# chalharu/rust-compression

Hardware: AMD Instinct MI355X
Metric: BZip2 level-9 encode MB/s (input bytes, HBM-resident in and out: the kernels' rate; value_end_to_end is host buffer to host buffer at the C ABI) (higher is better)
Workload: dtype u8/u32

## Files before the change

rust-compression_amd/csrc/k_bwt.hip:

```cpp
#include "bzgpu.h"
#include <algorithm>
#include <atomic>
#include <cstdio>
#include <cstdlib>
#include <vector>

namespace bzgpu {
constexpr u32 kGhSpan = 8;
constexpr u32 kSymSpan = 8;

enum { SRC_TEXT = 0, SRC_PAIRS = 1, SRC_MM = 2, SRC_WALK = 3, SRC_SURV = 4, SRC_LISTG = 5,
       SRC_TEXTK = 6, SRC_WALKK = 7, SRC_MMK = 8,
       SRC_MMC = 9,
       SRC_PERJ = 10,
       SRC_PACKED = 11,
       SRC_PERJK = 12,
       SRC_WALKA = 13 };
template <int SRC> struct src_is_list {
    static constexpr bool value = (SRC == SRC_PAIRS || SRC == SRC_SURV || SRC == SRC_LISTG || SRC == SRC_PERJ || SRC == SRC_PERJK || SRC == SRC_PACKED);
};

struct KeyInfo {
    u8 bits;
    u8 chars;
// ... 2547 lines not shown
__global__ __launch_bounds__(kSortThreads) void k_link_compact(BwtArgs a, const u32 *__restrict__ VS, u32 *__restrict__ Kout, u32 *__restrict__ Vout)
{
    constexpr u32 NW = kSortThreads / 64;
    __shared__ u32 s_off, s_wsum[NW];
    u32 tile, lb;
    xcd_remap(gridDim.x, a.nb, tile, lb);
    if (lb == 0xFFFFFFFFu) return;
    const u32 cnt = a.count2[lb];
    const u32 start = tile * kSortTile;
    const u32 ntiles = (cnt + kSortTile - 1) / kSortTile;
    if (tile == 0 && threadIdx.x == 0) {
        u32 tot = 0;
        for (u32 t = 0; t < ntiles; ++t) tot += a.tile_nf[lb * kTilesPerBlock + t];
        a.count[lb] = tot;
    }
    if (start >= cnt) return;
    const size_t base = (size_t)lb * kSlot;
    if (threadIdx.x == 0) {
        u32 off = 0;
        for (u32 t = 0; t < tile; ++t) off += a.tile_nf[lb * kTilesPerBlock + t];
        s_off = off;
    }
    const u8 *gb8 = group_bytes(a, lb);
    const u32 w = threadIdx.x >> 6, l = threadIdx.x & 63u;
    const u32 wbase = start + w * 1024u;
    u64 keep[16];
    u32 xv[16];
    u32 wcount = 0;
#pragma unroll
    for (u32 r = 0; r < 16; ++r) {
        const u32 idx = wbase + r * 64u + l;
        const u32 c = idx < cnt ? idx : cnt - 1u;
        xv[r] = ld_stream(VS + base + c);
        keep[r] = __ballot(idx < cnt && gb8[c] != 1u);
        wcount += (u32)__popcll(keep[r]);
    }
    if (l == 0) s_wsum[w] = wcount;
    __syncthreads();
    u32 off = s_off;
    for (u32 k = 0; k < w; ++k) off += s_wsum[k];
    const u64 lt_mask = (l == 0) ? 0ull : (~0ull >> (64 - l));
#pragma unroll
    for (u32 r = 0; r < 16; ++r) {
        if ((keep[r] >> l) & 1ull) {
            const u32 at = off + (u32)__popcll(keep[r] & lt_mask);
            Kout[base + at] = a.R[base + xv[r]] & ~kFinalBit;
            Vout[base + at] = xv[r];
        }
        off += (u32)__popcll(keep[r]);
    }
}

__global__ __launch_bounds__(kSortThreads) void k_period_mark(BwtArgs a, u32 step, const u32 *__restrict__ K,
                                                               const u32 *__restrict__ V, u8 *__restrict__ impure)
{
    u32 tile, lb;
    xcd_remap(gridDim.x, a.nb, tile, lb);
    if (lb == 0xFFFFFFFFu) return;
    const u32 cnt = a.count[lb];
    const u32 start = tile * kSortTile;
    if (start >= cnt || a.lin_p[(size_t)lb * kPerK] == 0u) return;
    const u32 n = a.blocks[lb].n;
    const u32 kmax = per_kmax(a);
    (void)step;
    const size_t base = (size_t)lb * kSlot;
    u32 lp[kPerK];
#pragma unroll
    for (u32 i = 0; i < kPerK; ++i) lp[i] = i < kmax ? a.lin_p[(size_t)lb * kPerK + i] : 0u;
    const u32 w = threadIdx.x >> 6, l = threadIdx.x & 63u;
    const u32 first = start + w * 1024u + l;
    u32 g[16], v[16];
#pragma unroll
    for (u32 r = 0; r < 16; ++r) {
        const u32 idx = first + r * 64u;
        const u32 c = idx < cnt ? idx : cnt - 1u;
        g[r] = ld_stream(K + base + c);
        v[r] = ld_stream(V + base + c);
    }
    u32 pg0 = 0, pv0 = 0;
    if (l == 0 && first > 0 && first < cnt) {
        pg0 = K[base + first - 1];
        pv0 = V[base + first - 1];
    }
    u32 lo[16], wh[16];
    u32 act = 0, vp_lo = 0;
#pragma unroll
    for (u32 r = 0; r < 16; ++r) {
        const u32 idx = first + r * 64u;
        u32 pg = wave_shr1(g[r]), pv = wave_shr1(v[r]);
        const u32 qg = (r == 0) ? pg0 : wave_lane(g[(r + 15) & 15], 63);
        const u32 qv = (r == 0) ? pv0 : wave_lane(v[(r + 15) & 15], 63);
        if (l == 0) {
            pg = qg;
            pv = qv;
        }
        lo[r] = v[r] < pv ? v[r] : pv;
        wh[r] = kPerK;
        if (idx < cnt && idx > 0 && g[r] == pg) {
            const u32 dist = v[r] < pv ? pv - v[r] : v[r] - pv;
#pragma unroll
            for (u32 i = 0; i < kPerK; ++i)
                if (lp[i] != 0u && lp[i] == dist) wh[r] = i;
            if (wh[r] == kPerK) impure[base + g[r]] = 1;
            else {
                act |= 1u << r;
                vp_lo |= (pv == lo[r] ? 1u : 0u) << r;
            }
        }
    }
    u64 here[16];
#pragma unroll
    for (u32 r = 0; r < 16; ++r) here[r] = ((act >> r) & 1u) ? (per_mis(a, lb, wh[r])[lo[r] >> 6] & (~0ull << (lo[r] & 63u))) : 1ull;
    u32 m[16];
#pragma unroll
    for (u32 r = 0; r < 16; ++r)
        m[r] = here[r] ? ((lo[r] >> 6) << 6) + (u32)__builtin_ctzll(here[r]) : per_nxt(a, lb, wh[r])[(lo[r] >> 6) + 1u];
    u64 ltw[16];
#pragma unroll
    for (u32 r = 0; r < 16; ++r) {
        if (m[r] >= n) m[r] -= n;
        ltw[r] = ((act >> r) & 1u) ? per_lt(a, lb, wh[r])[m[r] >> 6] : 0ull;
    }
#pragma unroll
    for (u32 r = 0; r < 16; ++r) {
        if (!((act >> r) & 1u)) continue;
        const bool lo_first = (ltw[r] >> (m[r] & 63u)) & 1ull;
        if (lo_first != (((vp_lo >> r) & 1u) != 0u)) impure[base + g[r]] = 1;
    }
}

__global__ __launch_bounds__(kSortThreads) void k_block_symbols(BwtArgs a, u32 *__restrict__ inuse_bits ,
                                                                u32 *__restrict__ pair_bits )
{
    __shared__ u32 s_bits[8];
    __shared__ u32 s_pair[kPairWords];
    u32 tile, lb;
    xcd_remap(gridDim.x, a.nb, tile, lb);
    if (lb == 0xFFFFFFFFu) return;
    const BlockDesc d = a.blocks[lb];
    const u32 n = d.n;
    constexpr u32 kSpan = kSymSpan * kSortTile;
    const u32 start = tile * kSpan;
    if (start >= n) return;
    const u8 *text = a.rle + d.rle_off;
    if (threadIdx.x < 8) s_bits[threadIdx.x] = 0;
    if (pair_bits)
        for (u32 i = threadIdx.x; i < kPairWords; i += kSortThreads) s_pair[i] = 0;
    __syncthreads();
    const u32 cnt = (n - start) < kSpan ? (n - start) : kSpan;
    const uintptr_t p0 = reinterpret_cast<uintptr_t>(text + start);
    const u32 lead = (u32)(p0 & 15u);
    const uint4 *src = reinterpret_cast<const uint4 *>(p0 - lead);
    const u32 t0 = text[0];
    u64 set[4] = {0, 0, 0, 0};
    for (u32 c = threadIdx.x; c * 16u < lead + cnt; c += kSortThreads) {
        const uint4 v = src[c];
        const u32 w[4] = {v.x, v.y, v.z, v.w};
        const u32 behind = start + c * 16u + 16u - lead;
        const u32 nxt = (pair_bits && behind < n) ? (u32)text[behind] : t0;
#pragma unroll
        for (u32 k = 0; k < 16; ++k) {
            const u32 pos = c * 16u + k;
            const u32 b = (w[k >> 2] >> ((k & 3u) * 8u)) & 0xFFu;
            const bool in = pos >= lead && pos < lead + cnt;
            const u64 bit = in ? (1ull << (b & 63u)) : 0ull;
            const u32 hi = b >> 6;
#pragma unroll
            for (u32 q = 0; q < 4; ++q) set[q] |= (hi == q) ? bit : 0ull;
            if (pair_bits && in) {
                u32 b2 = (k < 15u) ? ((w[(k + 1u) >> 2] >> (((k + 1u) & 3u) * 8u)) & 0xFFu) : nxt;
                if (start + (pos - lead) + 1u == n) b2 = t0;
                const u32 pr = (b << 8) | b2;
                if (!((s_pair[pr >> 5] >> (pr & 31u)) & 1u)) atomicOr(&s_pair[pr >> 5], 1u << (pr & 31u));
            }
        }
    }
    u32 seen[8];
#pragma unroll
    for (u32 q = 0; q < 4; ++q) {
        seen[2 * q] = (u32)set[q];
        seen[2 * q + 1] = (u32)(set[q] >> 32);
    }
#pragma unroll
    for (u32 q = 0; q < 8; ++q) {
        u32 v = seen[q];
#pragma unroll
        for (u32 dd = 32; dd >= 1; dd >>= 1) v |= __shfl_xor(v, dd, 64);
        if ((threadIdx.x & 63u) == 0 && v) atomicOr(&s_bits[q], v);
    }
    __syncthreads();
    if (threadIdx.x < 8 && s_bits[threadIdx.x]) atomicOr(&inuse_bits[lb * 8 + threadIdx.x], s_bits[threadIdx.x]);
    if (pair_bits)
        for (u32 i = threadIdx.x; i < kPairWords; i += kSortThreads)
            if (s_pair[i]) atomicOr(&pair_bits[(size_t)lb * kPairWords + i], s_pair[i]);
}

__global__ __launch_bounds__(256) void k_key_params(const u32 *__restrict__ inuse_bits, const u32 *__restrict__ pair_bits,
                                                     u8 *__restrict__ sym_code, u8 *__restrict__ keyinfo)
{
    __shared__ u32 s_pairs[4];
    const u32 lb = blockIdx.x;
    const u32 *bits = inuse_bits + lb * 8;
    const u32 v = threadIdx.x;
    u32 before = 0;
    for (u32 q = 0; q < (v >> 5); ++q) before += __popc(bits[q]);
    before += __popc(bits[v >> 5] & ((1u << (v & 31u)) - 1u));
    sym_code[(size_t)lb * 256 + v] = (u8)before;
    if (pair_bits) {
        u32 mine = 0;
        for (u32 i = v; i < kPairWords; i += 256u) mine += __popc(pair_bits[(size_t)lb * kPairWords + i]);
        mine = wave_incl_sum(mine);
        if ((v & 63u) == 63u) s_pairs[v >> 6] = mine;
    }
    __syncthreads();
    if (v == 0) {
        u32 alpha = 0;
        for (u32 q = 0; q < 8; ++q) alpha += __popc(bits[q]);
        u32 nbits = 1;
        while ((1u << nbits) < alpha) ++nbits;
        u32 chars = (nbits >= 8) ? 4u : 30u / nbits;
        if (chars > 8u) chars = 8u;
        KeyInfo ki;
        ki.bits = (u8)nbits;
        ki.chars = (u8)chars;
        ki.form = 0;
        ki.pad = 0;
        if (pair_bits) {
            const u32 npairs = s_pairs[0] + s_pairs[1] + s_pairs[2] + s_pairs[3];
            u32 pbits = 1;
            while (pbits < 11u && (1u << pbits) < npairs) ++pbits;
            const u32 cpair = 2u * (30u / pbits) < 8u ? 2u * (30u / pbits) : 8u;
            if (pbits <= 10u && cpair > chars) {
                ki.bits = (u8)pbits;
                ki.chars = (u8)cpair;
                ki.form = 1;
            }
        }
        reinterpret_cast<KeyInfo *>(keyinfo)[lb] = ki;
    }
}

__global__ __launch_bounds__(kSortThreads) void k_pack_text(BwtArgs a, u8 *__restrict__ ptext)
{
    __shared__ u8 s_code[256];
    __shared__ u32 s_out[kSortTile / 32 * 10];
    __shared__ u32 s_pair[kPairWords];
    __shared__ u16 s_before[kPairWords];
    __shared__ u32 s_wsum[kSortThreads / 64];
    __shared__ u32 s_hist[2][1024];
    u32 span, lb;
    xcd_remap(gridDim.x, a.nb, span, lb);
    if (lb == 0xFFFFFFFFu) return;
    const BlockDesc d = a.blocks[lb];
    const u32 n = d.n;
    const u32 start0 = span * kGhSpan * kSortTile;
    if (n == 0 || start0 >= n + 16u) return;
    const u8 *text = a.rle + d.rle_off;
    const KeyInfo ki = reinterpret_cast<const KeyInfo *>(a.keyinfo)[lb];
    const u32 bits = ki.bits;
    const bool pairs = ki.form != 0;
    const bool count = a.gh_tiles != nullptr && counts_from_pack(ki);
    if (count)
        for (u32 i = threadIdx.x; i < 2u * 1024u; i += kSortThreads) (&s_hist[0][0])[i] = 0;
    if (pairs) {
        static_assert(kPairWords == 4 * kSortThreads, "four words of the pair map per thread");
        const uint4 w4 = reinterpret_cast<const uint4 *>(a.pair_bits + (size_t)lb * kPairWords)[threadIdx.x];
        const u32 w[4] = {w4.x, w4.y, w4.z, w4.w};
        const u32 mine = __popc(w[0]) + __popc(w[1]) + __popc(w[2]) + __popc(w[3]);
        const u32 inc = wave_incl_sum(mine);
        if ((threadIdx.x & 63u) == 63u) s_wsum[threadIdx.x >> 6] = inc;
        __syncthreads();
        u32 run = inc - mine;
        for (u32 k = 0; k < (threadIdx.x >> 6); ++k) run += s_wsum[k];
#pragma unroll
        for (u32 q = 0; q < 4; ++q) {
            s_pair[threadIdx.x * 4u + q] = w[q];
            s_before[threadIdx.x * 4u + q] = (u16)run;
            run += __popc(w[q]);
        }
    } else {
        for (u32 i = threadIdx.x; i < 256; i += kSortThreads) s_code[i] = a.sym_code[(size_t)lb * 256 + i];
    }
    __syncthreads();
    u8 *s_bytes = reinterpret_cast<u8 *>(s_out);
    u32 *const hist = s_hist[threadIdx.x & 1u];
#pragma unroll 1
    for (u32 sp = 0; sp < kGhSpan; ++sp) {
        const u32 tile = span * kGhSpan + sp, start = tile * kSortTile;
        if (start >= n + 16u) break;
#pragma unroll
        for (u32 h = 0; h < 2; ++h) {
            const u32 g = h * kSortThreads + threadIdx.x;
            const u32 i0 = start + g * 8u;
            u32 lo = 0, hi = 0, ninth = 0;
            if (i0 + 9u <= n) {
                const uintptr_t p = reinterpret_cast<uintptr_t>(text + i0);
                const u32 *ap = reinterpret_cast<const u32 *>(p & ~(uintptr_t)3);
                const u32 w0 = ap[0], w1 = ap[1], w2 = ap[2];
                lo = __builtin_amdgcn_alignbyte(w1, w0, (u32)(p & 3u));
                hi = __builtin_amdgcn_alignbyte(w2, w1, (u32)(p & 3u));
                ninth = (w2 >> (8u * (u32)(p & 3u))) & 0xFFu;
            } else if (i0 < n + 16u) {
                for (u32 q = 0; q < 9; ++q) {
                    const u32 i = i0 + q;
                    const u32 c = (i < n + 16u + (q >> 3)) ? (u32)text[i < n ? i : (i - n) % n] : 0u;
                    if (q < 4) lo |= c << (8u * q);
                    else if (q < 8) hi |= c << (8u * (q - 4u));
                    else ninth = c;
                }
            }
            u64 va = 0, vb = 0;
#pragma unroll
            for (u32 q = 0; q < 8; ++q) {
                const u32 byte = ((q < 4 ? lo >> (8u * q) : hi >> (8u * (q - 4u)))) & 0xFFu;
                u32 code;
                if (pairs) {
                    const u32 b2 = q == 7 ? ninth : (((q + 1 < 4 ? lo >> (8u * (q + 1)) : hi >> (8u * (q + 1 - 4u)))) & 0xFFu);
                    const u32 pr = (byte << 8) | b2;
                    code = (u32)s_before[pr >> 5] + __popc(s_pair[pr >> 5] & ((1u << (pr & 31u)) - 1u));
                    if (i0 + q >= n + 16u) code = 0;
                    if (count && i0 + q < n) atomicAdd(&hist[code], 1u);
                } else {
                    code = s_code[byte];
                }
                if (q < 4) va = (va << bits) | (u64)code;
                else vb = (vb << bits) | (u64)code;
            }
            for (u32 k = 0; k < bits; ++k) {
                const u32 sh = 8u * (bits - 1u - k), half = 4u * bits;
                u32 o = sh >= half ? (u32)(va >> (sh - half)) : ((u32)(vb >> sh) | (u32)(va << (half - sh)));
                s_bytes[g * bits + k] = (u8)o;
            }
        }
        __syncthreads();
        u32 *dst = reinterpret_cast<u32 *>(ptext + (size_t)lb * kPtSlot + (size_t)tile * 1024u * bits);
        for (u32 i = threadIdx.x; i < 256u * bits; i += kSortThreads) dst[i] = s_out[i];
        __syncthreads();
    }
    if (count) {
        u32 *out = a.gh_tiles + ((size_t)lb * kTilesPerBlock + span) * 3 * kMaxBins;
        for (u32 i = threadIdx.x; i < 1024u; i += kSortThreads) out[i] = s_hist[0][i] + s_hist[1][i];
    }
}

int KernelProf::begin(hipStream_t st, int id, u64 nbytes)
{
    if (!on) return -1;
// ... 519 lines not shown
```

rust-compression_amd/csrc/k_huff.hip:

```cpp
#include "bzgpu.h"
#include <cstdlib>

namespace bzgpu {

constexpr u32 kHuffThreads = 512;

__device__ __forceinline__ u32 weight_add(u32 x, u32 y)
{
    const u32 dx = x & 0xFFu, dy = y & 0xFFu;
    return ((x & 0xFFFFFF00u) + (y & 0xFFFFFF00u)) | (1u + (dx > dy ? dx : dy));
}

__device__ void down_heap(u32 *buf, u32 nn, u32 len)
{
    const u32 tmp = buf[nn];
    u32 leaf = (nn << 1) + 1;
    while (leaf < len) {
        if (leaf + 1 < len && buf[buf[leaf]] > buf[buf[leaf + 1]]) leaf += 1;
        if (buf[tmp] < buf[buf[leaf]]) break;
        buf[nn] = buf[leaf];
        nn = leaf;
        leaf = (nn << 1) + 1;
    }
    buf[nn] = tmp;
// ... 737 lines not shown
#pragma unroll
    for (int t = 0; t < 6; ++t) last[t] = -1000000;
    for (u32 g = g_lo; g < g_hi; ++g) {
        const u32 v = selector[g];
#pragma unroll
        for (int t = 0; t < 6; ++t)
            if ((u32)t == v) last[t] = (int)g;
    }
    int start_last[6];
#pragma unroll
    for (int t = 0; t < 6; ++t) {
        const int inc = wave_incl_max32(last[t]);
        if (lane == 63) s_scan[wave] = (u32)inc;
        __syncthreads();
        int carry = -1000000;
        for (u32 k = 0; k < wave; ++k) carry = (int)s_scan[k] > carry ? (int)s_scan[k] : carry;
        const int prev = __shfl_up(inc, 1, 64);
        int ex = (lane == 0) ? -1000000 : prev;
        ex = ex > carry ? ex : carry;
        start_last[t] = (ex < 0) ? -(t + 1) : ex;
        __syncthreads();
    }
    u32 my_bits = 0;
    {
        int cur[6];
#pragma unroll
        for (int t = 0; t < 6; ++t) cur[t] = start_last[t];
        for (u32 g = g_lo; g < g_hi; ++g) {
            const u32 v = selector[g];
            int lv = 0;
#pragma unroll
            for (int t = 0; t < 6; ++t)
                if ((u32)t == v) lv = cur[t];
            u32 pos = 0;
#pragma unroll
            for (int t = 0; t < 6; ++t) pos += (cur[t] > lv) ? 1u : 0u;
#pragma unroll
            for (int t = 0; t < 6; ++t)
                if ((u32)t == v) cur[t] = (int)g;
            my_bits += pos + 1u;
        }
    }
    u32 sel_off, sel_total;
    {
        const u32 inc = wave_incl_sum(my_bits);
        if (lane == 63) s_scan[wave] = inc;
        __syncthreads();
        u32 carry = 0, tot = 0;
        for (u32 k = 0; k < kHuffThreads / 64; ++k) {
            if (k < wave) carry += s_scan[k];
            tot += s_scan[k];
        }
        sel_off = carry + inc - my_bits;
        sel_total = tot;
        __syncthreads();
    }
    const u32 tab_bit0 = sel_bit0 + sel_total;
    if (tab_lane) {
        const u8 *l = s_len[tb];
        u32 nb = 5, curr = l[0];
        for (u32 i = 0; i < alpha; ++i) {
            const u32 li = l[i];
            nb += 2u * (li > curr ? li - curr : curr - li) + 1u;
            curr = li;
        }
        s_first[tb][0] = nb;
    }
    __syncthreads();
    u32 tab_off[7];
    tab_off[0] = tab_bit0;
    for (u32 t = 0; t < 6; ++t) tab_off[t + 1] = tab_off[t] + (t < group_num ? s_first[t][0] : 0u);
    const u32 hb = tab_off[group_num];
    for (u32 w = tid; w <= (hb >> 5); w += kHuffThreads) stream[w] = 0;
    __syncthreads();
    auto put = [&](u32 bitpos, u32 v, u32 nbits) {
        const u32 w = bitpos >> 5, o = bitpos & 31u;
        const unsigned long long x = (unsigned long long)v << (64u - o - nbits);
        atomicOr(&stream[w], (u32)(x >> 32));
        if ((u32)x) atomicOr(&stream[w + 1], (u32)x);
    };
    if (tid == 0) {
        put(0, 0x314159u, 24);
        put(24, 0x265359u, 24);
        put(48, a.crc[lb], 32);
        put(81, a.orig_ptr[lb], 24);
        put(105, in_use16, 16);
        u32 bp = 121;
        for (u32 i = 0; i < 16; ++i) {
            const u32 half = (ubits[i >> 1] >> ((i & 1u) * 16u)) & 0xFFFFu;
            if (half) {
                put(bp, __brev(half) >> 16, 16);
                bp += 16;
            }
        }
        put(bp, group_num, 3);
        put(bp + 3, n_selectors, 15);
    }
    {
        int cur[6];
#pragma unroll
        for (int t = 0; t < 6; ++t) cur[t] = start_last[t];
        u32 bp = sel_bit0 + sel_off;
        for (u32 g = g_lo; g < g_hi; ++g) {
            const u32 v = selector[g];
            int lv = 0;
#pragma unroll
            for (int t = 0; t < 6; ++t)
                if ((u32)t == v) lv = cur[t];
            u32 pos = 0;
#pragma unroll
            for (int t = 0; t < 6; ++t) pos += (cur[t] > lv) ? 1u : 0u;
#pragma unroll
            for (int t = 0; t < 6; ++t)
                if ((u32)t == v) cur[t] = (int)g;
            put(bp, (1u << (pos + 1u)) - 2u, pos + 1u);
            bp += pos + 1u;
        }
    }
    if (tab_lane) {
        const u8 *l = s_len[tb];
        u32 bp = tab_off[tb];
        u32 curr = l[0];
        put(bp, curr, 5);
        bp += 5;
        for (u32 i = 0; i < alpha; ++i) {
            const u32 li = l[i];
            while (curr < li) { put(bp, 2, 2); bp += 2; curr += 1; }
            while (curr > li) { put(bp, 3, 2); bp += 2; curr -= 1; }
            bp += 1;
        }
    }
    if (tid == 0) {
        bo.header_bits = hb;
        bo.pad = used_ranges | (sel_total << 5);
        bo.total_bits = (u64)hb + payload_bits;
        bo.group_num = group_num;
        bo.n_selectors = n_selectors;
        bo.max_len = max_len;
        bo.lm_tables = s_lm[0] + s_lm[1] + s_lm[2] + s_lm[3] + s_lm[4] + s_lm[5];
        bo.crc = a.crc[lb];
        bo.orig_ptr = a.orig_ptr[lb];
        if ((u64)hb + payload_bits + 96u > (u64)kStreamWords * 32u) atomicExch(a.error_flag, 1u);
    }
    {
        const u64 tb = (u64)hb + payload_bits;
        u32 w0 = (hb >> 5) + 1u;
        u32 w1 = (u32)(tb >> 5) + 2u;
        if (w1 > kStreamWords) w1 = kStreamWords;
        for (u32 w = w0 + tid; w < w1; w += kHuffThreads) stream[w] = 0;
    }
    BZ_HT(3)
}

__global__ __launch_bounds__(256) void k_emit_payload(HuffArgs a)
{
    __shared__ u32 s_code[6 * kMaxAlpha];
    __shared__ u32 s_sym[256 * kGSize / 2];
    const u32 lb = blockIdx.y;
    const BlockOut &bo = a.out[lb];
    const u32 mtf_count = bo.mtf_count;
    const u32 n_selectors = bo.n_selectors;
    const u32 g0 = blockIdx.x * 256u;
    if (g0 >= n_selectors) return;
    const u32 *code_len = a.code_len + (size_t)lb * 6 * kMaxAlpha;
    for (u32 i = threadIdx.x; i < 6 * kMaxAlpha; i += 256u) s_code[i] = code_len[i];
    const u16 *mtf = a.mtf + (size_t)lb * a.mtf_stride;
    stage_symbols(s_sym, mtf, g0, mtf_count);
    __syncthreads();
    const u32 g = g0 + threadIdx.x;
    if (g >= n_selectors) return;
    const u32 gs = g * kGSize;
    const u32 cnt = (gs + kGSize < mtf_count) ? kGSize : mtf_count - gs;
    const u32 *my = s_sym + threadIdx.x * (kGSize / 2);
    const u32 *tab = s_code + (u32)a.selector[(size_t)lb * kSelStride + g] * kMaxAlpha;
    const u32 bitpos = bo.header_bits + a.group_bitoff[(size_t)lb * kGboStride + g];
    u32 *stream = a.stream + (size_t)lb * kStreamWords;
    u32 widx = bitpos >> 5;
    u32 nacc = bitpos & 31u;
    u64 acc = 0;
    bool first = true;
    for (u32 i = 0; i < cnt; ++i) {
        const u32 cl = tab[(my[i >> 1] >> ((i & 1u) * 16u)) & 0xFFFFu];
        const u32 len = cl >> 24, code = cl & 0xFFFFFFu;
        acc |= (u64)code << (64u - nacc - len);
        nacc += len;
        if (nacc >= 32u) {
            const u32 word = (u32)(acc >> 32);
            if (first) {
                atomicOr(&stream[widx], word);
                first = false;
            } else {
                stream[widx] = word;
            }
            ++widx;
            acc <<= 32;
            nacc -= 32u;
        }
    }
    if (nacc) atomicOr(&stream[widx], (u32)(acc >> 32));
}

constexpr u32 kSweepThreads = 256;
constexpr u32 kSweepTilesX = 11;
constexpr u32 kTabArena = 6 * (3 * kMaxAlpha + 4);

__device__ __forceinline__ u32 huff_group_num(u32 mtf_count)
{
    if (mtf_count < 200) return 2;
    if (mtf_count < 600) return 3;
    if (mtf_count < 1200) return 4;
    if (mtf_count < 2400) return 5;
    return 6;
}

__device__ __forceinline__ void lm_wave_sync()
{
    __builtin_amdgcn_fence(__ATOMIC_ACQ_REL, "workgroup");
    __builtin_amdgcn_wave_barrier();
}
__device__ void lm_code_lengths_wave(const u32 *rfreq, u32 n, u32 *scr, u32 scr_words, u32 row, u8 *out, u32 lane)
{
    const u32 lim = kLim;
    u32 *map = scr;
    u32 *sfreq = map + kMaxAlpha;
    u32 *c = sfreq + kMaxAlpha;
    u32 *misc = c + kMaxAlpha;
    u32 *max_elem = misc, *b = misc + 20, *cur = misc + 40;
    u32 *val = misc + 64 + kMaxAlpha;
    u32 *ty = val + lim * row;
    u32 *w = scr + scr_words - kMaxAlpha;
    for (u32 i = lane; i < n; i += 64u) {
        const u32 f = rfreq[i];
        w[i] = (f > 1u ? f : 1u) << 8;
    }
    lm_wave_sync();
    for (u32 i = lane; i < n; i += 64u) {
        const u32 f = w[i];
        u32 r = 0;
        for (u32 q = 0; q < n; ++q) {
            const u32 x = w[q];
            r += (x > f || (x == f && q < i)) ? 1u : 0u;
        }
        sfreq[r] = f;
        map[r] = i;
    }
    if (lane == 0) {
        for (u32 j = 0; j < lim; ++j) { max_elem[j] = 0; b[j] = 0; cur[j] = 0; }
        u32 excess = (1u << lim) - n;
        const u32 half = 1u << (lim - 1);
        max_elem[lim - 1] = n;
        for (u32 j = 0; j < lim; ++j) {
            if (excess >= half) {
                b[j] = 1;
                excess -= half;
            }
            excess <<= 1;
            if (lim >= 2 + j) max_elem[lim - 2 - j] = max_elem[lim - 1 - j] / 2 + n;
        }
        max_elem[0] = b[0];
        for (u32 j = 1; j < lim; ++j)
            if (max_elem[j] > 2 * max_elem[j - 1] + b[j]) max_elem[j] = 2 * max_elem[j - 1] + b[j];
    }
    lm_wave_sync();
    for (u32 j = 0; j < lim; ++j)
        for (u32 t = lane; t < max_elem[j]; t += 64u) { val[j * row + t] = 0; ty[j * row + t] = 0; }
    for (u32 i = lane; i < n; i += 64u) c[i] = lim;
    lm_wave_sync();
    for (u32 t = lane; t < n && t < max_elem[lim - 1]; t += 64u) {
        val[(lim - 1) * row + t] = sfreq[t];
        ty[(lim - 1) * row + t] = t;
    }
    if (lane == 0 && b[lim - 1] == 1) {
        c[0] -= 1;
        cur[lim - 1] += 1;
    }
    lm_wave_sync();
    const u32 last_leaf = sfreq[n - 1];
    for (u32 j = lim - 1; j > 0;) {
        const u32 next0 = cur[j], me = max_elem[j], cap = max_elem[j - 1];
        const u32 K = (me > next0 + 1u) ? (me - next0) / 2u : 0u;
        u32 *vj = val + j * row, *dv = val + (j - 1) * row, *dt = ty + (j - 1) * row;
        for (u32 k0 = 0; k0 < K; k0 += 64u) {
            const u32 k = k0 + lane;
            u32 pk = 0;
            if (k < K) pk = weight_add(vj[next0 + 2u * k], vj[next0 + 2u * k + 1u]);
            lm_wave_sync();
            if (k < K) vj[k] = pk;
        }
        lm_wave_sync();
        for (u32 k = lane; k < K; k += 64u) {
            const u32 pk = vj[k];
            if (pk > last_leaf) {
                u32 lo = 0, hi = n;
                while (lo < hi) {
                    const u32 mid = (lo + hi) >> 1;
                    if (sfreq[mid] >= pk) lo = mid + 1u;
                    else hi = mid;
                }
                const u32 pos = k + lo;
                if (pos < cap) {
                    dv[pos] = pk;
                    dt[pos] = n;
                }
            }
        }
        for (u32 i = lane; i < n; i += 64u) {
            const u32 sf = sfreq[i];
            u32 lo = 0, hi = K;
            while (lo < hi) {
                const u32 mid = (lo + hi) >> 1;
                if (vj[mid] > sf) lo = mid + 1u;
                else hi = mid;
            }
            const u32 pos = i + lo;
            if (pos < cap) {
                dv[pos] = sf;
                dt[pos] = i;
            }
        }
        lm_wave_sync();
        j -= 1;
        if (lane == 0) cur[j] = 0;
        lm_wave_sync();
        if (b[j] == 1) {
            u32 need = 1;
            for (u32 li = j; need > 0u && li < lim; ++li) {
                const u32 c0 = cur[li];
                u32 npk = 0;
                for (u32 t0 = 0; t0 < need; t0 += 64u) {
                    const u32 t = t0 + lane;
                    bool isp = false;
                    if (t < need) {
                        const u32 x = ty[li * row + c0 + t];
                        if (x == n) isp = true;
                        else c[x] -= 1;
                    }
                    npk += (u32)__popcll(__ballot(isp));
                }
                lm_wave_sync();
                if (lane == 0) cur[li] = c0 + need;
                need = 2u * npk;
                lm_wave_sync();
            }
        }
        lm_wave_sync();
    }
    for (u32 i = lane; i < n; i += 64u) out[map[i]] = (u8)c[i];
    lm_wave_sync();
}

template <u32 THREADS>
__device__ __forceinline__ void stage_symbols_n(u32 *s_sym, const u16 *__restrict__ mtf, u32 g0, u32 mtf_count)
// ... 575 lines not shown
```

Before: 15070.

## Stage Huffman payload in LDS and split pair-bit scan from symbol-set scan

k_emit_payload now packs each workgroup's bit span into a shared-memory buffer and writes it to global memory with aligned 16-byte stores. Only the two boundary words use atomicOr, replacing per-thread scattered global atomics and stores. The code-length lookups are also batched ten at a time, with a padding entry in the table so there is no per-symbol branch. The BWT symbol-usage kernel gets a separate pair_bits path that derives the in-use bitmap from pair-table rows with a ballot, dropping the 64-bit set accumulation on that path. The cost is more LDS and extra barriers, plus an error flag if a span overflows the buffer.

```diff
diff --git a/rust-compression_amd/csrc/k_bwt.hip b/rust-compression_amd/csrc/k_bwt.hip
--- a/rust-compression_amd/csrc/k_bwt.hip
+++ b/rust-compression_amd/csrc/k_bwt.hip
@@ -2723,12 +2723,45 @@
     const u32 lead = (u32)(p0 & 15u);
     const uint4 *src = reinterpret_cast<const uint4 *>(p0 - lead);
     const u32 t0 = text[0];
+    if (pair_bits) {
+        for (u32 c = threadIdx.x; c * 16u < lead + cnt; c += kSortThreads) {
+            const uint4 v = src[c];
+            const u32 w[4] = {v.x, v.y, v.z, v.w};
+            const u32 behind = start + c * 16u + 16u - lead;
+            const u32 nxt = (behind < n) ? (u32)text[behind] : t0;
+#pragma unroll
+            for (u32 k = 0; k < 16; ++k) {
+                const u32 pos = c * 16u + k;
+                if (pos < lead || pos >= lead + cnt) continue;
+                const u32 b = (w[k >> 2] >> ((k & 3u) * 8u)) & 0xFFu;
+                u32 b2 = (k < 15u) ? ((w[(k + 1u) >> 2] >> (((k + 1u) & 3u) * 8u)) & 0xFFu) : nxt;
+                if (start + (pos - lead) + 1u == n) b2 = t0;
+                const u32 pr = (b << 8) | b2;
+                if (!((s_pair[pr >> 5] >> (pr & 31u)) & 1u)) atomicOr(&s_pair[pr >> 5], 1u << (pr & 31u));
+            }
+        }
+        __syncthreads();
+        for (u32 b0 = 0; b0 < 256u; b0 += kSortThreads) {
+            const u32 b = b0 + threadIdx.x;
+            u32 row = 0;
+            if (b < 256u) {
+#pragma unroll
+                for (u32 q = 0; q < 8; ++q) row |= s_pair[8u * b + q];
+            }
+            const u64 m = __ballot(row != 0u);
+            if ((threadIdx.x & 63u) == 0 && b < 256u) {
+                if ((u32)m) atomicOr(&inuse_bits[lb * 8 + (b >> 5)], (u32)m);
+                if ((u32)(m >> 32)) atomicOr(&inuse_bits[lb * 8 + (b >> 5) + 1u], (u32)(m >> 32));
+            }
+        }
+        for (u32 i = threadIdx.x; i < kPairWords; i += kSortThreads)
+            if (s_pair[i]) atomicOr(&pair_bits[(size_t)lb * kPairWords + i], s_pair[i]);
+        return;
+    }
     u64 set[4] = {0, 0, 0, 0};
     for (u32 c = threadIdx.x; c * 16u < lead + cnt; c += kSortThreads) {
         const uint4 v = src[c];
         const u32 w[4] = {v.x, v.y, v.z, v.w};
-        const u32 behind = start + c * 16u + 16u - lead;
-        const u32 nxt = (pair_bits && behind < n) ? (u32)text[behind] : t0;
 #pragma unroll
         for (u32 k = 0; k < 16; ++k) {
             const u32 pos = c * 16u + k;
@@ -2738,12 +2771,6 @@
             const u32 hi = b >> 6;
 #pragma unroll
             for (u32 q = 0; q < 4; ++q) set[q] |= (hi == q) ? bit : 0ull;
-            if (pair_bits && in) {
-                u32 b2 = (k < 15u) ? ((w[(k + 1u) >> 2] >> (((k + 1u) & 3u) * 8u)) & 0xFFu) : nxt;
-                if (start + (pos - lead) + 1u == n) b2 = t0;
-                const u32 pr = (b << 8) | b2;
-                if (!((s_pair[pr >> 5] >> (pr & 31u)) & 1u)) atomicOr(&s_pair[pr >> 5], 1u << (pr & 31u));
-            }
         }
     }
     u32 seen[8];
@@ -2761,9 +2788,6 @@
     }
     __syncthreads();
     if (threadIdx.x < 8 && s_bits[threadIdx.x]) atomicOr(&inuse_bits[lb * 8 + threadIdx.x], s_bits[threadIdx.x]);
-    if (pair_bits)
-        for (u32 i = threadIdx.x; i < kPairWords; i += kSortThreads)
-            if (s_pair[i]) atomicOr(&pair_bits[(size_t)lb * kPairWords + i], s_pair[i]);
 }
 
 __global__ __launch_bounds__(256) void k_key_params(const u32 *__restrict__ inuse_bits, const u32 *__restrict__ pair_bits,
diff --git a/rust-compression_amd/csrc/k_huff.hip b/rust-compression_amd/csrc/k_huff.hip
--- a/rust-compression_amd/csrc/k_huff.hip
+++ b/rust-compression_amd/csrc/k_huff.hip
@@ -913,52 +913,104 @@
     BZ_HT(3)
 }
 
-__global__ __launch_bounds__(256) void k_emit_payload(HuffArgs a)
-{
-    __shared__ u32 s_code[6 * kMaxAlpha];
-    __shared__ u32 s_sym[256 * kGSize / 2];
-    const u32 lb = blockIdx.y;
+constexpr u32 kEmitThreads = 256;
+constexpr u32 kEmitBufWords = kEmitThreads * kGSize * kLim / 32u + 1u + 3u;
+static_assert(kEmitThreads * kGSize * kLim % 32u == 0 && kEmitBufWords % 4u == 0, "the span buffer is whole 16-byte pieces");
+static_assert(kEmitBufWords >= kEmitThreads * kGSize / 2, "the span buffer first holds the staged symbols");
+
+__global__ __launch_bounds__(kEmitThreads) void k_emit_payload(HuffArgs a)
+{
+    __shared__ u32 s_code[6 * kMaxAlpha + 1];
+    __shared__ __attribute__((aligned(16))) u32 s_buf[kEmitBufWords];
+    const u32 lb = blockIdx.y, tid = threadIdx.x;
     const BlockOut &bo = a.out[lb];
     const u32 mtf_count = bo.mtf_count;
     const u32 n_selectors = bo.n_selectors;
-    const u32 g0 = blockIdx.x * 256u;
+    const u32 g0 = blockIdx.x * kEmitThreads;
     if (g0 >= n_selectors) return;
     const u32 *code_len = a.code_len + (size_t)lb * 6 * kMaxAlpha;
-    for (u32 i = threadIdx.x; i < 6 * kMaxAlpha; i += 256u) s_code[i] = code_len[i];
+    for (u32 i = tid; i < 6 * kMaxAlpha; i += kEmitThreads) s_code[i] = code_len[i];
+    if (tid == 0) s_code[6 * kMaxAlpha] = 0;
     const u16 *mtf = a.mtf + (size_t)lb * a.mtf_stride;
-    stage_symbols(s_sym, mtf, g0, mtf_count);
-    __syncthreads();
-    const u32 g = g0 + threadIdx.x;
-    if (g >= n_selectors) return;
+    stage_symbols(s_buf, mtf, g0, mtf_count);
+    const u32 *gbo = a.group_bitoff + (size_t)lb * kGboStride;
+    const u32 hb = bo.header_bits;
+    const u32 g1 = g0 + kEmitThreads;
+    const u32 lo = hb + gbo[g0];
+    const u32 hi = (g1 < n_selectors) ? hb + gbo[g1] : (u32)bo.total_bits;
+    if (hi <= lo) return;
+    u32 *stream = a.stream + (size_t)lb * kStreamWords;
+    const u32 wf = lo >> 5, wl = (hi - 1u) >> 5;
+    const u32 base = wf - ((wf + (u32)((reinterpret_cast<uintptr_t>(stream) >> 2) & 3u)) & 3u);
+    const u32 nwords = wl - base + 1u;
+    if (nwords > kEmitBufWords) {
+        if (tid == 0) atomicExch(a.error_flag, 1u);
+        return;
+    }
+    const u32 g = g0 + tid;
+    const bool live = g < n_selectors;
     const u32 gs = g * kGSize;
-    const u32 cnt = (gs + kGSize < mtf_count) ? kGSize : mtf_count - gs;
-    const u32 *my = s_sym + threadIdx.x * (kGSize / 2);
-    const u32 *tab = s_code + (u32)a.selector[(size_t)lb * kSelStride + g] * kMaxAlpha;
-    const u32 bitpos = bo.header_bits + a.group_bitoff[(size_t)lb * kGboStride + g];
-    u32 *stream = a.stream + (size_t)lb * kStreamWords;
-    u32 widx = bitpos >> 5;
-    u32 nacc = bitpos & 31u;
-    u64 acc = 0;
-    bool first = true;
-    for (u32 i = 0; i < cnt; ++i) {
-        const u32 cl = tab[(my[i >> 1] >> ((i & 1u) * 16u)) & 0xFFFFu];
-        const u32 len = cl >> 24, code = cl & 0xFFFFFFu;
-        acc |= (u64)code << (64u - nacc - len);
-        nacc += len;
-        if (nacc >= 32u) {
-            const u32 word = (u32)(acc >> 32);
-            if (first) {
-                atomicOr(&stream[widx], word);
-                first = false;
-            } else {
-                stream[widx] = word;
-            }
-            ++widx;
-            acc <<= 32;
-            nacc -= 32u;
-        }
-    }
-    if (nacc) atomicOr(&stream[widx], (u32)(acc >> 32));
+    const u32 cnt = !live ? 0u : (gs + kGSize < mtf_count) ? kGSize : mtf_count - gs;
+    __syncthreads();
+    u32 sym[kGSize / 2];
+#pragma unroll
+    for (u32 k = 0; k < kGSize / 2; ++k) sym[k] = s_buf[tid * (kGSize / 2) + k];
+    __syncthreads();
+    for (u32 q = tid * 4u; q < nwords; q += kEmitThreads * 4u) *reinterpret_cast<uint4 *>(s_buf + q) = make_uint4(0, 0, 0, 0);
+    __syncthreads();
+    if (live) {
+        const u32 tab = (u32)a.selector[(size_t)lb * kSelStride + g] * kMaxAlpha;
+        const u32 bitpos = hb + gbo[g];
+        u32 widx = (bitpos >> 5) - base;
+        u32 nacc = bitpos & 31u;
+        u64 acc = 0;
+        bool first = true;
+#pragma unroll
+        for (u32 k0 = 0; k0 < kGSize / 2; k0 += 5) {
+            u32 cl[10];
+#pragma unroll
+            for (u32 j = 0; j < 10; ++j) {
+                const u32 i = 2u * k0 + j;
+                const u32 s = (sym[i >> 1] >> ((i & 1u) * 16u)) & 0xFFFFu;
+                cl[j] = s_code[(i < cnt) ? tab + s : 6u * kMaxAlpha];
+            }
+#pragma unroll
+            for (u32 j = 0; j < 10; ++j) {
+                const u32 len = cl[j] >> 24, code = cl[j] & 0xFFFFFFu;
+                acc |= (u64)code << ((64u - nacc - len) & 63u);
+                nacc += len;
+                if (nacc >= 32u) {
+                    const u32 word = (u32)(acc >> 32);
+                    if (first) {
+                        atomicOr(&s_buf[widx], word);
+                        first = false;
+                    } else {
+                        s_buf[widx] = word;
+                    }
+                    ++widx;
+                    acc <<= 32;
+                    nacc -= 32u;
+                }
+            }
+        }
+        if (nacc) atomicOr(&s_buf[widx], (u32)(acc >> 32));
+    }
+    __syncthreads();
+    for (u32 q = tid * 4u; q < nwords; q += kEmitThreads * 4u) {
+        const u32 w = base + q;
+        if (w > wf && w + 3u < wl && w + 3u < kStreamWords) {
+            *reinterpret_cast<uint4 *>(stream + w) = *reinterpret_cast<const uint4 *>(s_buf + q);
+            continue;
+        }
+#pragma unroll
+        for (u32 j = 0; j < 4; ++j) {
+            const u32 ww = w + j;
+            if (ww < wf || ww > wl || ww >= kStreamWords) continue;
+            const u32 v = s_buf[q + j];
+            if (ww != wf && ww != wl) stream[ww] = v;
+            else if (v) atomicOr(&stream[ww], v);
+        }
+    }
 }
 
 constexpr u32 kSweepThreads = 256;
```

Measured after the change: 15350 (median of 6 runs). 1.8% higher.
